# augustgw/early-exit-transformer

Hardware: AMD Instinct MI355X
Metric: mel-frames/sec encoder forward (all exits) + summed per-exit CTC loss, d_model=256 12-layer (higher is better)
Workload: dtype fp16x3 (hi/lo-split fp16 MFMA operands, three products per GEMM, fp32 accumulate; v_mfma_f32_16x16x32_f16)

## Files before the change

### early_exit_transformer_amd/csrc/eec_device.h

```cpp
#pragma once
#include <hip/hip_runtime.h>
#include <stdint.h>

namespace eec {

typedef _Float16 half_t;
typedef _Float16 h8 __attribute__((ext_vector_type(8)));
typedef _Float16 h4 __attribute__((ext_vector_type(4)));
typedef _Float16 h2 __attribute__((ext_vector_type(2)));
typedef float f32x16 __attribute__((ext_vector_type(16)));
typedef float f32x4 __attribute__((ext_vector_type(4)));

#ifndef EEC_OPERAND_BF16
#define EEC_OPERAND_BF16 0
#endif
typedef __bf16 bf8_t __attribute__((ext_vector_type(8)));
typedef __bf16 bf2_t __attribute__((ext_vector_type(2)));
typedef float f32x2_t __attribute__((ext_vector_type(2)));

constexpr int kWave = 64;
constexpr float kLnEps = 1e-5f;
constexpr float kLog2e = 1.4426950408889634f;
constexpr float kHalfMax = 65504.0f;

// ... 318 lines not shown
template <int MT, int NT>
__device__ __forceinline__ void accs_q_to_std(f32x16 (&acc)[MT][NT]) {
  asm volatile("s_nop 7\n\ts_nop 7\n\ts_nop 2" ::: "memory");
#pragma unroll
  for (int a = 0; a < MT; ++a)
#pragma unroll
    for (int b = 0; b < NT; ++b) acc_q_to_std(acc[a][b]);
}
template <int MT, int NT>
__device__ __forceinline__ void accs_std_to_q(f32x16 (&acc)[MT][NT]) {
#pragma unroll
  for (int a = 0; a < MT; ++a)
#pragma unroll
    for (int b = 0; b < NT; ++b) acc_std_to_q(acc[a][b]);
}
__device__ __forceinline__ const char* a_lane16(const char* a_lane, int ld_bytes) {
  const int lane = lane_id(), hh = lane >> 5, u = (lane >> 4) & 1;
  return a_lane + u * (16 - 16 * ld_bytes) + hh * 16;
}
__device__ __forceinline__ const uint4* w_lane16(const uint4* w_lane) {
  const int lane = lane_id(), hh = lane >> 5, u = (lane >> 4) & 1;
  return w_lane + 96 * hh + 16 * u;
}

struct WAddr16 {
  const char* base;
  __device__ __forceinline__ uint4 load(size_t uniform_u4) const { return *(const uint4*)(base + uniform_u4 * 16); }
};
__device__ __forceinline__ WAddr16 w_addr16(const uint4* w_lane) {
  const int lane = lane_id(), hh = lane >> 5, u = (lane >> 4) & 1;
  return WAddr16{(const char*)(w_lane + 96 * hh + 16 * u)};
}

template <int NP, int PF, int NT>
__device__ __forceinline__ void ring_fill_16(WRing<NP, PF, NT>& r, const uint4* __restrict__ w_lane, size_t nt_stride, int steps_avail) {
  static_assert(PF % 2 == 0, "the ring is dealt in double k-steps");
  const WAddr16 w16 = w_addr16(w_lane);
#pragma unroll
  for (int p = 0; p < PF; ++p)
    if (p < steps_avail) {
#pragma unroll
      for (int nt = 0; nt < NT; ++nt) {
        r.q[p][nt][0] = w16.load(nt * nt_stride + 16 * (p & 1) + (size_t)(p >> 1) * 256);
        if (NP == 3) r.q[p][nt][(NP == 3) ? 1 : 0] = w16.load(nt * nt_stride + 16 * (p & 1) + (size_t)(p >> 1) * 256 + 64);
      }
    }
  __builtin_amdgcn_sched_barrier(0);
}

__device__ __forceinline__ void quad_mac16(f32x16& acc, int ra, int cb, h8 a, h8 b) {
  const int q = 4 * (2 * ra + cb);
  f32x4 t = {acc[q], acc[q + 1], acc[q + 2], acc[q + 3]};
  t = mfma32(a, b, t);
  acc[q] = t[0], acc[q + 1] = t[1], acc[q + 2] = t[2], acc[q + 3] = t[3];
}
template <int NP, int KS, int NT, bool SWAP, int PF, typename Side = NoSide, int SIDE_VALU = 0, int MT = 2, bool IN_STD = true, bool OUT_STD = true>
__device__ __forceinline__ void gemm_ring_16(f32x16 (&acc)[MT][NT], const char* a_lane, int ld_bytes, int plane_bytes,
                                             const uint4* __restrict__ w_lane, size_t nt_stride, WRing<NP, PF, NT>& r, Side side = Side()) {
  static_assert(KS % 2 == 0 && PF % 2 == 0, "double k-steps");
  constexpr int LO = (NP == 3) ? 1 : 0;
  const char* a16 = a_lane16(a_lane, ld_bytes);
  const WAddr16 w16 = w_addr16(w_lane);
  if constexpr (IN_STD) accs_std_to_q<MT, NT>(acc);
  h8 ah[2][MT], al[2][MT];
#pragma unroll
  for (int mt = 0; mt < MT; ++mt) {
    ah[0][mt] = *(const h8*)(a16 + mt * 32 * ld_bytes);
    if (NP == 3) al[0][mt] = *(const h8*)(a16 + plane_bytes + mt * 32 * ld_bytes);
  }
#pragma unroll
  for (int p = 0; p < KS; ++p) {
    const int S = p >> 1, rb = p & 1, cur = p & 1, nxt = cur ^ 1;
    if (p + 1 < KS) {
      const int off = (16 * ((p + 1) & 1)) * ld_bytes + ((p + 1) >> 1) * 64;
#pragma unroll
      for (int mt = 0; mt < MT; ++mt) {
        ah[nxt][mt] = *(const h8*)(a16 + mt * 32 * ld_bytes + off);
        if (NP == 3) al[nxt][mt] = *(const h8*)(a16 + plane_bytes + mt * 32 * ld_bytes + off);
      }
      __builtin_amdgcn_sched_barrier(0);
    }
#pragma unroll
    for (int wb = 0; wb < 2; ++wb) {
#pragma unroll
      for (int nt = 0; nt < NT; ++nt) {
        const h8 bh = __builtin_bit_cast(h8, r.q[(2 * S + wb) % PF][nt][0]);
        const h8 bl = __builtin_bit_cast(h8, r.q[(2 * S + wb) % PF][nt][LO]);
#pragma unroll
        for (int pr = (NP == 3 ? 0 : 2); pr < 3; ++pr)
#pragma unroll
          for (int mt = 0; mt < MT; ++mt) {
            const h8 a = pr == 0 ? al[cur][mt] : ah[cur][mt], w = pr == 1 ? bl : bh;
            if (!SWAP) quad_mac16(acc[mt][nt], rb, wb, a, w);
            else quad_mac16(acc[mt][nt], wb, rb, w, a);
          }
        if (rb == 1) {
          if (2 * S + PF < KS) {
            r.q[(2 * S + wb) % PF][nt][0] = w16.load(nt * nt_stride + 16 * wb + (size_t)(S + PF / 2) * 256);
            if (NP == 3) r.q[(2 * S + wb) % PF][nt][LO] = w16.load(nt * nt_stride + 16 * wb + (size_t)(S + PF / 2) * 256 + 64);
          }
        }
      }
    }
    side(p);
    if (SIDE_VALU > 0) {
#pragma unroll
      for (int i = 0; i < MT * NT * NP; ++i) {
        __builtin_amdgcn_sched_group_barrier(0x008, 2, 0);
        __builtin_amdgcn_sched_group_barrier(0x002, SIDE_VALU, 0);
      }
    }
    __builtin_amdgcn_sched_barrier(0);
#ifdef EEC_KSTEP_STAMPS
    if (NT == 2) eec_kstep_stamp();
#endif
  }
  if constexpr (OUT_STD) accs_q_to_std<MT, NT>(acc);
}

template <int NP, int NT, bool SWAP, int MT = 2, bool IN_STD = true, bool OUT_STD = true>
__device__ __forceinline__ void gemm_plain_16(f32x16 (&acc)[MT][NT], const char* a_lane, int ld_bytes, int plane_bytes,
                                              const uint4* __restrict__ w_lane, size_t nt_stride, int ks) {
  const char* a16 = a_lane16(a_lane, ld_bytes);
  const uint4* w16 = w_lane16(w_lane);
  if constexpr (IN_STD) accs_std_to_q<MT, NT>(acc);
  for (int S = 0; S < ks / 2; ++S) {
#pragma unroll
    for (int nt = 0; nt < NT; ++nt) {
      h8 bh[2], bl[2];
#pragma unroll
      for (int rb = 0; rb < 2; ++rb) {
        bh[rb] = __builtin_bit_cast(h8, w16[nt * nt_stride + 16 * rb + (size_t)S * 256]);
        bl[rb] = bh[rb];
        if (NP == 3) bl[rb] = __builtin_bit_cast(h8, w16[nt * nt_stride + 16 * rb + (size_t)S * 256 + 64]);
      }
#pragma unroll
      for (int mt = 0; mt < MT; ++mt) {
        h8 ah[2], al[2];
#pragma unroll
        for (int rb = 0; rb < 2; ++rb) {
          ah[rb] = *(const h8*)(a16 + (mt * 32 + 16 * rb) * ld_bytes + S * 64);
          al[rb] = ah[rb];
          if (NP == 3) al[rb] = *(const h8*)(a16 + plane_bytes + (mt * 32 + 16 * rb) * ld_bytes + S * 64);
        }
        if (NP == 3) {
          if (SWAP) tile_mac16(acc[mt][nt], bh, al), tile_mac16(acc[mt][nt], bl, ah);
          else tile_mac16(acc[mt][nt], al, bh), tile_mac16(acc[mt][nt], ah, bl);
        }
        if (SWAP) tile_mac16(acc[mt][nt], bh, ah);
        else tile_mac16(acc[mt][nt], ah, bh);
      }
    }
  }
  if constexpr (OUT_STD) accs_q_to_std<MT, NT>(acc);
}

template <int NP>
constexpr bool kMfma16For = NP == 3 || (EEC_MFMA16_NP1 != 0 && NP == 1);
template <int NP, int PF, int NT>
__device__ __forceinline__ void ring_fill(WRing<NP, PF, NT>& r, const uint4* __restrict__ w_lane, size_t nt_stride, int steps_avail) {
  if constexpr (kMfma16For<NP>) ring_fill_16<NP, PF, NT>(r, w_lane, nt_stride, steps_avail);
  else ring_fill_32<NP, PF, NT>(r, w_lane, nt_stride, steps_avail);
}
template <int NP, int KS, int NT, bool SWAP, int PF, typename Side = NoSide, int SIDE_VALU = 0, int MT = 2, bool IN_STD = true, bool OUT_STD = true>
__device__ __forceinline__ void gemm_ring(f32x16 (&acc)[MT][NT], const char* a_lane, int ld_bytes, int plane_bytes,
                                          const uint4* __restrict__ w_lane, size_t nt_stride, WRing<NP, PF, NT>& r, Side side = Side()) {
  if constexpr (kMfma16For<NP>) gemm_ring_16<NP, KS, NT, SWAP, PF, Side, SIDE_VALU, MT, IN_STD, OUT_STD>(acc, a_lane, ld_bytes, plane_bytes, w_lane, nt_stride, r, side);
  else gemm_ring_32<NP, KS, NT, SWAP, PF, Side, SIDE_VALU, MT>(acc, a_lane, ld_bytes, plane_bytes, w_lane, nt_stride, r, side);
}
template <int NP, int NT, bool SWAP, int MT = 2, bool IN_STD = true, bool OUT_STD = true>
__device__ __forceinline__ void gemm_plain(f32x16 (&acc)[MT][NT], const char* a_lane, int ld_bytes, int plane_bytes,
                                           const uint4* __restrict__ w_lane, size_t nt_stride, int ks) {
  if constexpr (kMfma16For<NP>) gemm_plain_16<NP, NT, SWAP, MT, IN_STD, OUT_STD>(acc, a_lane, ld_bytes, plane_bytes, w_lane, nt_stride, ks);
  else gemm_plain_32<NP, NT, SWAP, MT>(acc, a_lane, ld_bytes, plane_bytes, w_lane, nt_stride, ks);
}

typedef int i32x8 __attribute__((ext_vector_type(8)));
constexpr int kE8M0One = 127;
constexpr float kF8WLoGain = 1.09f;
constexpr float kF8ALoGain = 1.17f;
__device__ __forceinline__ h2 lo8_gain(h2 lo) {
  const h2 g = {(half_t)kF8ALoGain, (half_t)kF8ALoGain};
  return lo * g;
}

__device__ __forceinline__ uint2 top_bytes(uint4 f) {
  return make_uint2(__builtin_amdgcn_perm(f.y, f.x, 0x07050301u), __builtin_amdgcn_perm(f.w, f.z, 0x07050301u));
}
__device__ __forceinline__ f32x16 mfma_f8(i32x8 a, i32x8 b, f32x16 c, int scale_a, int scale_b) {
  return __builtin_amdgcn_mfma_scale_f32_32x32x64_f8f6f4(a, b, c, 1 , 1 , 0, scale_a, 0, scale_b);
}
__device__ __forceinline__ int lo8_pos(int k) {
  return (k & ~63) + 32 * ((k >> 3) & 1) + 8 * ((k >> 4) & 3) + (k & 7);
}

constexpr int kF8Rec = 400;
template <int NT>
struct WGroupF8 {
  uint4 lo[NT][2];
  int sc[NT];
// ... 304 lines not shown
```

### early_exit_transformer_amd/csrc/ffn.hip

```cpp
#ifdef EEC_FFN_TRAIN_BWD
#define EEC_OPERAND_BF16 1
#endif
#if defined(EEC_FFN_TRAIN) || defined(EEC_FFN_TRAIN_BWD)
#define EEC_MFMA16_NP1 1
#endif
#include "eec_blocks.h"
#include "eec_drop.h"

namespace eec {

constexpr int kFfnThreads = 512;
constexpr int kFC = 128;
constexpr int kHLd = (kFC + 8) * 2;
template <int D>
struct FfnGeo {
  using G = Geo<D>;
  static constexpr int kHPlane = G::kRows * kHLd;
  static constexpr int kNT2 = D / 128;
  static constexpr int kLds = 2 * G::kAPlane + (4 * kHPlane > G::kETile ? 4 * kHPlane : G::kETile);
};
#ifndef EEC_TR_NT
#define EEC_TR_NT 1
#endif
#if defined(EEC_FFN_TRAIN_BWD) && !defined(EEC_PF1_NP3)
// ... 148 lines not shown
  const int lane = lane_id(), w = wave_id();
  const int hh = lane >> 5, wl = w & 3;
  const int w_s = wave_id_sgpr();
  const int wl_s = w_s & 3;
  const bool is_producer = w < 4;
  const int row0 = row_tile_index() * G::kRows;
  const int M = a.M, F = a.F;
  float* __restrict__ x = a.x;
  char* lds_h = smem + 2 * kAPlane;
  char* lds_e = lds_h;
  const char* a_lane = smem + (lane & 31) * kALd + hh * 16;

  const int nft = F / 32;
  const int nchunk = (nft + 3) / 4;
  const int ks2_total = F / 16;
#ifndef EEC_SKEW
#define EEC_SKEW 56
#endif
#ifndef EEC_WARM_SLOTS
#define EEC_WARM_SLOTS 4
#endif
  auto phys = [&](int c) { return c >= nchunk ? c - nchunk : c; };
  const size_t w2_nt_stride = (size_t)ks2_total * 128;

#ifdef EEC_TIMELINE
  int tl_idx = 0;
#endif
  TL_STAMP();
#if EEC_SKEW > 0
  for (int i = 0; i < (int)((blockIdx.x >> 3) & 3); ++i) __builtin_amdgcn_s_sleep(EEC_SKEW);
#endif
  constexpr int RNP = NP == 8 ? 1 : NP;
  constexpr bool Q16 = kMfma16For<NP>;
  auto run = [&](auto prod_tag) {
  constexpr bool producer = decltype(prod_tag)::value;
  [[maybe_unused]] const eect::DropState ds_act(eect::Drop{TR ? a.tr.p : 0.0f, a.tr.seed, a.tr.site_act});
  WRing<RNP, kPF1, 1> r1;
  WRing<RNP, kPF2, NTP> r2;
  WGroupF8<1> wg1[kNW1];
  WGroupF8<NTP> wg2[kNW2];
  const size_t w2f8_nt = (size_t)(F / 64) * kF8Rec;
  auto w1f8_lane = [&](const WPtrs& W, int ft) { return W.w1f8 + (size_t)ft * (D / 64) * kF8Rec + lane; };
  auto w2f8_lane = [&](const WPtrs& W, int c, int h = 0) {
    return W.w2f8 + ((size_t)(NT2 * wl + NTP * h) * (F / 64) + 2 * c) * kF8Rec + lane;
  };
  auto fill1 = [&](const WPtrs& W, int ft) {
    if constexpr (NP == 8) {
      ring_fill_f8<kPF1, 1>(r1, w1f8_lane(W, ft), 0);
#pragma unroll
      for (int g = 0; g < kNW1; ++g) f8_group_load<1>(wg1[g], w1f8_lane(W, ft) + (size_t)g * kF8Rec, 0);
    } else {
      ring_fill<RNP, kPF1, 1>(r1, W.w1p + (size_t)ft * nts + lane, 0, KS);
    }
  };
  auto fill2 = [&](const WPtrs& W, int c) {
    if constexpr (NP == 8) {
      ring_fill_f8<kPF2, NTP>(r2, w2f8_lane(W, c), w2f8_nt);
#pragma unroll
      for (int g = 0; g < kNW2; ++g) f8_group_load<NTP>(wg2[g], w2f8_lane(W, c) + (size_t)g * kF8Rec, w2f8_nt);
    } else {
      ring_fill<RNP, kPF2, NTP>(r2, W.w2p + ((size_t)(NT2 * wl) * ks2_total + c * (kFC / 16)) * 128 + lane, w2_nt_stride,
                             min(kFC / 16, ks2_total - c * (kFC / 16)));
    }
  };
  auto start_streams = [&](const WPtrs& W) {
    if constexpr (producer) {
// ... 128 lines not shown
        const int row = row0 + w * RPW + i;
        v[i] = zero_row<G::kQ>();
        if (row < M) v[i] = load_row<D>(x + (size_t)row * D, lane);
      }
      __builtin_amdgcn_sched_barrier(0);
      start_streams(W0);
      float mu[RPW], rs[RPW];
      layer_norm_rows<D, RPW>(v, lg, lb, mu, rs);
#pragma unroll
      for (int i = 0; i < RPW; ++i) {
        const int row = row0 + w * RPW + i;
        if (row < M) {
          store_row<D>(a.tr.ln + (size_t)row * D, v[i], lane);
          if (lane == 0) a.tr.mean[row] = mu[i], a.tr.rstd[row] = rs[i];
        }
      }
      rows_to_planes<D, NP, RPW>(smem, v, w * RPW, row0, M, true);
    } else {
      rows_f32_to_planes<D, NP, true>(smem, x, row0, M, a.st[0].ln_g, a.st[0].ln_b, [&]() { start_streams(W0); });
    }
  }
  TL_STAMP();
  __syncthreads();
  TL_STAMP();

  [[maybe_unused]] ProjStream<(QNP ? QNP : 1), kLPF, NW> rq;
  unsigned sink = 0;
  const int nslots = nchunk + 2;
  f32x16 acc2c[NH][MT][NTP];
  static_for<NS>([&](auto si_tag) {
    constexpr int si = decltype(si_tag)::value;
    const WPtrs W = wptrs(si);
    const float* __restrict__ b1s = EEC_STAGE_FIELD(si, b1);
    if constexpr (producer) {
      [[maybe_unused]] f32x16 preq[TR == 2 ? MT : 1];
      [[maybe_unused]] auto request_pre = [&](int hcol0) {
#pragma unroll
        for (int mt = 0; mt < MT; ++mt)
#pragma unroll
          for (int g = 0; g < 4; ++g) {
            const int frame = Q16 ? mt * 32 + 16 * (g & 1) + (lane & 15) : mt * 32 + (lane & 31);
            const int hid = Q16 ? wl * 32 + 16 * (g >> 1) + 8 * hh + 4 * ((lane >> 4) & 1) : wl * 32 + 4 * hh + g * 8;
            const int row = min(row0 + frame, M - 1);
            typedef float f32x4_t __attribute__((ext_vector_type(4)));
            const f32x4_t v = __builtin_nontemporal_load((const f32x4_t*)(a.tr.pre + (size_t)row * F + hcol0 + hid));
            preq[mt][4 * g] = v[0], preq[mt][4 * g + 1] = v[1], preq[mt][4 * g + 2] = v[2], preq[mt][4 * g + 3] = v[3];
          }
      };
      auto silu_pair = [&](const f32x16 (&acc)[MT][1], char* hb, int step, h2& keep_hi, h2& keep_lo, [[maybe_unused]] int hcol0 = 0) {
        const int mt = step >> 3, q = step & 7;
        const float u0 = acc[mt][0][2 * q], u1 = acc[mt][0][2 * q + 1];
        if constexpr (TR == 2) {
          const float x0 = preq[mt][2 * q], x1 = preq[mt][2 * q + 1];
          const float sg0 = __builtin_amdgcn_rcpf(1.0f + __builtin_amdgcn_exp2f(-kLog2e * x0));
          const float sg1 = __builtin_amdgcn_rcpf(1.0f + __builtin_amdgcn_exp2f(-kLog2e * x1));
          const float t0 = u0 * sg0 * (1.0f + x0 * (1.0f - sg0)), t1 = u1 * sg1 * (1.0f + x1 * (1.0f - sg1));
          if ((q & 1) == 0) {
            keep_hi = __builtin_bit_cast(h2, t0);
            keep_lo = __builtin_bit_cast(h2, t1);
            return;
          }
          const int g = q >> 1;
          const int frame = Q16 ? mt * 32 + 16 * (g & 1) + (lane & 15) : mt * 32 + (lane & 31);
          const int hid = Q16 ? wl * 32 + 16 * (g >> 1) + 8 * hh + 4 * ((lane >> 4) & 1) : wl * 32 + 4 * hh + g * 8;
          const int row = row0 + frame;
          const size_t idx = (size_t)row * F + hcol0 + hid;
          float m[4];
          ds_act.mul4(idx, m);
          const float d0 = __builtin_bit_cast(float, keep_hi) * m[0], d1 = __builtin_bit_cast(float, keep_lo) * m[1], d2 = t0 * m[2], d3 = t1 * m[3];
          if (row < M) tape_store4(a.tr.act + idx, d0, d1, d2, d3);
          constexpr int SNPT = NP == 1 ? 1 : 3;
          const hl2_t sa = split2<SNPT>(d0, d1), sb = split2<SNPT>(d2, d3);
          char* dst = hb + frame * kHLd + hid * 2;
          h4 hi, lo;
          hi.xy = sa.hi, hi.zw = sb.hi, lo.xy = sa.lo, lo.zw = sb.lo;
          *(h4*)dst = hi;
          if (NP == 3) *(h4*)(dst + kHPlane) = lo;
          return;
        }
        if constexpr (TR == 1) {
          const float s0 = silu_f(u0), s1 = silu_f(u1);
          if ((q & 1) == 0) {
            keep_hi = __builtin_bit_cast(h2, s0);
            keep_lo = __builtin_bit_cast(h2, s1);
            return;
          }
          const int g = q >> 1;
          const int frame = Q16 ? mt * 32 + 16 * (g & 1) + (lane & 15) : mt * 32 + (lane & 31);
          const int hid = Q16 ? wl * 32 + 16 * (g >> 1) + 8 * hh + 4 * ((lane >> 4) & 1) : wl * 32 + 4 * hh + g * 8;
          const int row = row0 + frame;
          const size_t idx = (size_t)row * F + hcol0 + hid;
          float m[4];
          ds_act.mul4(idx, m);
          const float h0 = __builtin_bit_cast(float, keep_hi) * m[0], h1 = __builtin_bit_cast(float, keep_lo) * m[1], h2v = s0 * m[2], h3 = s1 * m[3];
          if (row < M) {
            tape_store4(a.tr.pre + idx, acc[mt][0][2 * q - 2], acc[mt][0][2 * q - 1], u0, u1);
            tape_store4(a.tr.act + idx, h0, h1, h2v, h3);
          }
          constexpr int SNPT = NP == 1 ? 1 : 3;
          const hl2_t sa = split2<SNPT>(h0, h1), sb = split2<SNPT>(h2v, h3);
          char* dst = hb + frame * kHLd + hid * 2;
          h4 hi, lo;
          hi.xy = sa.hi, hi.zw = sb.hi, lo.xy = sa.lo, lo.zw = sb.lo;
          *(h4*)dst = hi;
          if (NP == 3) *(h4*)(dst + kHPlane) = lo;
          return;
        }
        constexpr int SNP = NP == 1 ? 1 : 3;
        const hl2_t sp = ACT == 0 ? split2<SNP>(silu_exp2(u0), silu_exp2(u1)) : split2<SNP>(fmaxf(u0, 0.f), fmaxf(u1, 0.f));
        if ((q & 1) == 0) {
          keep_hi = sp.hi;
          keep_lo = sp.lo;
        } else {
          const int g = q >> 1;
          const int frame = Q16 ? mt * 32 + 16 * (g & 1) + (lane & 15) : mt * 32 + (lane & 31);
          const int hid = Q16 ? wl * 32 + 16 * (g >> 1) + 8 * hh + 4 * ((lane >> 4) & 1) : wl * 32 + 4 * hh + g * 8;
          char* dst = hb + frame * kHLd + hid * 2;
          h4 hi, lo;
          hi.xy = keep_hi, hi.zw = sp.hi, lo.xy = keep_lo, lo.zw = sp.lo;
          *(h4*)dst = hi;
          if (NP == 3) *(h4*)(dst + kHPlane) = lo;
          if (NP == 8) {
            h4 lg;
            lg.xy = lo8_gain(keep_lo), lg.zw = lo8_gain(sp.lo);
            const uint2 lb = __builtin_bit_cast(uint2, lg);
            *(unsigned*)(hb + kHPlane + (mt * 32 + (lane & 31)) * kH8Ld + lo8_pos(wl * 32 + 4 * hh + (q >> 1) * 8)) =
                __builtin_amdgcn_perm(lb.y, lb.x, 0x07050301u);
          }
        }
      };
      auto init_bias = [&](f32x16 (&acc)[MT][1], int ft) {
        if constexpr (TR == 2) {
          zero_acc(acc);
          return;
        }
        if constexpr (Q16) {
          const int u = (lane >> 4) & 1;
#pragma unroll
          for (int ra = 0; ra < 2; ++ra) {
            const float4 bb = *(const float4*)(b1s + ft * 32 + 16 * ra + 8 * hh + 4 * u);
#pragma unroll
            for (int mt = 0; mt < MT; ++mt)
#pragma unroll
              for (int cb = 0; cb < 2; ++cb) {
                acc[mt][0][4 * (2 * ra + cb) + 0] = bb.x;
                acc[mt][0][4 * (2 * ra + cb) + 1] = bb.y;
                acc[mt][0][4 * (2 * ra + cb) + 2] = bb.z;
                acc[mt][0][4 * (2 * ra + cb) + 3] = bb.w;
              }
          }
          return;
        }
#pragma unroll
        for (int g = 0; g < 4; ++g) {
          const float4 bb = *(const float4*)(b1s + ft * 32 + 8 * g + 4 * hh);
#pragma unroll
          for (int mt = 0; mt < MT; ++mt) {
            acc[mt][0][4 * g + 0] = bb.x;
            acc[mt][0][4 * g + 1] = bb.y;
            acc[mt][0][4 * g + 2] = bb.z;
            acc[mt][0][4 * g + 3] = bb.w;
          }
        }
      };
      constexpr int kSideEvery = KS / (8 * MT);
      auto slot = [&](int s, f32x16 (&cur)[MT][1], f32x16 (&prev)[MT][1]) {
        const int ft = (s < nchunk ? phys(s) : s) * 4 + wl;
        const bool do_gemm = s < nchunk && ft < nft;
        const bool do_silu = s >= 1 && s - 1 < nchunk && phys(s - 1) * 4 + wl < nft;
        char* hb_prev = lds_h + ((s - 1) & 1) * 2 * kHPlane;
        [[maybe_unused]] const int hcol_prev = do_silu ? phys(s - 1) * kFC : 0;
        h2 khi, klo;
        if (do_gemm) {
          init_bias(cur, ft);
          const uint4* w1_lane = W.w1p + (size_t)ft * nts + lane;
          const char* a8_lane = smem + kAPlane + (lane & 31) * kA8Ld + hh * 32;
          if (do_silu) {
            auto side = [&](int st) {
              if (st % kSideEvery == 0) silu_pair(prev, hb_prev, st / kSideEvery, khi, klo, hcol_prev);
            };
            if constexpr (NP == 8)
              gemm_ring_f8<D / 64, 1, true, kPF1, decltype(side), EEC_SIDE_VALU_NP8, kNW1, MT>(
                  cur, a_lane, kALd, a8_lane, kA8Ld, w1f8_lane(W, ft), 0, r1, wg1, side);
            else
              gemm_ring<RNP, KS, 1, true, kPF1, decltype(side), (NP == 3 ? EEC_SIDE_VALU_NP3 : 7), MT, !Q16, !Q16>(cur, a_lane, kALd, kAPlane, w1_lane,
                                                                                                  0, r1, side);
          } else {
            if constexpr (NP == 8)
              gemm_ring_f8<D / 64, 1, true, kPF1, NoSide, 0, kNW1, MT>(cur, a_lane, kALd, a8_lane, kA8Ld,
                                                                                                                    w1f8_lane(W, ft), 0, r1, wg1);
            else
              gemm_ring<RNP, KS, 1, true, kPF1, NoSide, 0, MT, !Q16, !Q16>(cur, a_lane, kALd, kAPlane, w1_lane, 0, r1);
          }
          if (s + 1 < nchunk && phys(s + 1) * 4 + wl < nft) fill1(W, phys(s + 1) * 4 + wl);
          if constexpr (TR == 2) request_pre(phys(s) * kFC);
        } else if (do_silu) {
#pragma unroll
          for (int st = 0; st < 8 * MT; ++st) silu_pair(prev, hb_prev, st, khi, klo, hcol_prev);
        }
        TL_STAMP();
        __syncthreads();
        TL_STAMP();
      };
      f32x16 accA[MT][1], accB[MT][1];
      for (int s = 0; s < nslots; s += 2) {
        slot(s, accA, accB);
        if (s + 1 < nslots) slot(s + 1, accB, accA);
      }
    } else {
#pragma unroll
      for (int h = 0; h < NH; ++h) zero_acc(acc2c[h]);
#if EEC_WARM_SLOTS > 0
      unsigned warm[4] = {0u, 0u, 0u, 0u};
#endif
      for (int s = 0; s < nslots; ++s) {
#if EEC_WARM_SLOTS > 0
        if (s == nslots - EEC_WARM_SLOTS) {
          const int lane_t = fresh_lane();
          if constexpr (si + 1 < NS) {
            const WPtrs Wn = wptrs(si + 1);
            const size_t wbytes = NP == 8 ? (size_t)(F / 32) * (D / 64) * kF8Rec * 16 : (size_t)F * D * 2 * (NP == 3 ? 2 : 1);
#pragma unroll
            for (int j = 0; j < 2; ++j) {
              warm[j] = touch_share(NP == 8 ? (const void*)Wn.w1f8 : (const void*)Wn.w1p, wbytes, wl_s, j, lane_t);
              warm[2 + j] = touch_share(NP == 8 ? (const void*)Wn.w2f8 : (const void*)Wn.w2p, wbytes, wl_s, j, lane_t);
            }
          } else if constexpr (QNP != 0) {
            warm[0] = QNP == 8 ? touch_share(a.qkv.wf8, (size_t)(3 * D / 32) * (D / 64) * kF8Rec * 16, wl_s, 0, lane_t)
                               : touch_share(a.qkv.wp, (size_t)3 * D * D * 2 * (QNP == 3 ? 2 : 1), wl_s, 0, lane_t);
          }
        }
#endif
        if (s >= 2) {
          const int cl = s - 2, c = phys(cl);
          const char* h_lane = lds_h + (cl & 1) * 2 * kHPlane + (lane & 31) * kHLd + hh * 16;
          const int ks2 = min(kFC / 16, ks2_total - c * (kFC / 16));
          const uint4* w2_lane = W.w2p + ((size_t)(NT2 * wl) * ks2_total + c * (kFC / 16)) * 128 + lane;
          if constexpr (NP == 8) {
            const char* h8_lane = lds_h + (cl & 1) * 2 * kHPlane + kHPlane + (lane & 31) * kH8Ld + hh * 32;
            if constexpr (NH == 1) {
              gemm_ring_f8<2, NTP, false, kPF2, NoSide, 0, kNW2, MT>(acc2c[0], h_lane, kHLd, h8_lane, kH8Ld, w2f8_lane(W, c), w2f8_nt, r2, wg2);
            } else {
#pragma unroll
              for (int h = 0; h < NH; ++h) {
                const uint4* next = h + 1 < NH ? w2f8_lane(W, c, h + 1) : (cl + 1 < nchunk ? w2f8_lane(W, phys(cl + 1), 0) : nullptr);
                gemm_ring_f8<2, NTP, false, kPF2, NoSide, 0, kNW2, MT, true>(acc2c[h], h_lane, kHLd, h8_lane, kH8Ld, w2f8_lane(W, c, h), w2f8_nt, r2, wg2, NoSide(), next);
              }
            }
          } else if (ks2 == kFC / 16) {
            gemm_ring<RNP, kFC / 16, NTP, false, kPF2, NoSide, 0, MT, !Q16, !Q16>(acc2c[0], h_lane, kHLd, kHPlane, w2_lane, w2_nt_stride, r2);
          } else {
            gemm_plain<RNP, NTP, false, MT, !Q16, !Q16>(acc2c[0], h_lane, kHLd, kHPlane, w2_lane, w2_nt_stride, ks2);
          }
          if (NH == 1 && cl + 1 < nchunk) fill2(W, phys(cl + 1));
        }
        TL_STAMP();
        __syncthreads();
        TL_STAMP();
      }
#if EEC_WARM_SLOTS > 0
      sink ^= warm[0] ^ warm[1] ^ warm[2] ^ warm[3];
#endif
    }
    const int lane_e = fresh_lane(), w_e = w_s;
    RowV<G::kQ> xr[RPW];
#pragma unroll
    for (int i = 0; i < RPW; ++i) {
      const int row = row0 + w_e * RPW + i;
      xr[i] = zero_row<G::kQ>();
      if (TR != 2 && row < M) xr[i] = load_row<D>(x + (size_t)row * D, lane_e);
    }
    __builtin_amdgcn_sched_barrier(0);
    constexpr bool more = si + 1 < NS;
    TL_STAMP();
    if constexpr (!producer) {
      if constexpr (Q16) {
#pragma unroll
        for (int h = 0; h < NH; ++h) accs_q_to_std<MT, NTP>(acc2c[h]);
      }
#pragma unroll
      for (int h = 0; h < NH; ++h)
        acc_to_etile<MT, NTP>(lds_e, G::kELd, acc2c[h], wl_s * 32 * NT2 + h * 32 * NTP, EEC_STAGE_FIELD(si, b2), lane_e);
    }
    TL_STAMP();
    if constexpr (more) {
      start_streams(wptrs(1));
    } else if constexpr (QNP != 0) {
      proj_fill<D, QNP, kLPF, NW>(rq, WMat{a.qkv.wp, a.qkv.wf8}, NW * w);
    }
    __syncthreads();
    TL_STAMP();
// ... 240 lines not shown
```

Baseline: 19.03 million.

## Split first FFN chunk's GEMM1 across producer and consumer waves by weight half

Adds a WBM mask to the 16x16x32 ring GEMM so a caller can compute only one half of the weight row-blocks. In the FFN kernel's fp16x3 path, the first slot's up-projection is split: producer waves compute the even half while consumer waves, which would otherwise sit idle during the first two slots, compute the odd half and apply SiLU to their part of the hidden tile. This is meant to shorten the pipeline fill latency at the start of each stage. The cost is more code paths, extra registers in the consumer, and an extra split of the SiLU work and sync logic, which could raise register pressure.

```diff
diff --git a/early_exit_transformer_amd/csrc/eec_device.h b/early_exit_transformer_amd/csrc/eec_device.h
--- a/early_exit_transformer_amd/csrc/eec_device.h
+++ b/early_exit_transformer_amd/csrc/eec_device.h
@@ -374,13 +374,13 @@
   return WAddr16{(const char*)(w_lane + 96 * hh + 16 * u)};
 }
 
-template <int NP, int PF, int NT>
+template <int NP, int PF, int NT, int WBM = 3>
 __device__ __forceinline__ void ring_fill_16(WRing<NP, PF, NT>& r, const uint4* __restrict__ w_lane, size_t nt_stride, int steps_avail) {
   static_assert(PF % 2 == 0, "the ring is dealt in double k-steps");
   const WAddr16 w16 = w_addr16(w_lane);
 #pragma unroll
   for (int p = 0; p < PF; ++p)
-    if (p < steps_avail) {
+    if (((WBM >> (p & 1)) & 1) && p < steps_avail) {
 #pragma unroll
       for (int nt = 0; nt < NT; ++nt) {
         r.q[p][nt][0] = w16.load(nt * nt_stride + 16 * (p & 1) + (size_t)(p >> 1) * 256);
@@ -396,7 +396,8 @@
   t = mfma32(a, b, t);
   acc[q] = t[0], acc[q + 1] = t[1], acc[q + 2] = t[2], acc[q + 3] = t[3];
 }
-template <int NP, int KS, int NT, bool SWAP, int PF, typename Side = NoSide, int SIDE_VALU = 0, int MT = 2, bool IN_STD = true, bool OUT_STD = true>
+template <int NP, int KS, int NT, bool SWAP, int PF, typename Side = NoSide, int SIDE_VALU = 0, int MT = 2, bool IN_STD = true, bool OUT_STD = true,
+          int WBM = 3>
 __device__ __forceinline__ void gemm_ring_16(f32x16 (&acc)[MT][NT], const char* a_lane, int ld_bytes, int plane_bytes,
                                              const uint4* __restrict__ w_lane, size_t nt_stride, WRing<NP, PF, NT>& r, Side side = Side()) {
   static_assert(KS % 2 == 0 && PF % 2 == 0, "double k-steps");
@@ -424,6 +425,7 @@
     }
 #pragma unroll
     for (int wb = 0; wb < 2; ++wb) {
+      if (!((WBM >> wb) & 1)) continue;
 #pragma unroll
       for (int nt = 0; nt < NT; ++nt) {
         const h8 bh = __builtin_bit_cast(h8, r.q[(2 * S + wb) % PF][nt][0]);
@@ -447,7 +449,7 @@
     side(p);
     if (SIDE_VALU > 0) {
 #pragma unroll
-      for (int i = 0; i < MT * NT * NP; ++i) {
+      for (int i = 0; i < MT * NT * NP * (WBM == 3 ? 2 : 1) / 2; ++i) {
         __builtin_amdgcn_sched_group_barrier(0x008, 2, 0);
         __builtin_amdgcn_sched_group_barrier(0x002, SIDE_VALU, 0);
       }
@@ -499,15 +501,18 @@
 
 template <int NP>
 constexpr bool kMfma16For = NP == 3 || (EEC_MFMA16_NP1 != 0 && NP == 1);
-template <int NP, int PF, int NT>
+template <int NP, int PF, int NT, int WBM = 3>
 __device__ __forceinline__ void ring_fill(WRing<NP, PF, NT>& r, const uint4* __restrict__ w_lane, size_t nt_stride, int steps_avail) {
-  if constexpr (kMfma16For<NP>) ring_fill_16<NP, PF, NT>(r, w_lane, nt_stride, steps_avail);
+  static_assert(WBM == 3 || kMfma16For<NP>, "weight row-block halves: 16x16x32 forms only");
+  if constexpr (kMfma16For<NP>) ring_fill_16<NP, PF, NT, WBM>(r, w_lane, nt_stride, steps_avail);
   else ring_fill_32<NP, PF, NT>(r, w_lane, nt_stride, steps_avail);
 }
-template <int NP, int KS, int NT, bool SWAP, int PF, typename Side = NoSide, int SIDE_VALU = 0, int MT = 2, bool IN_STD = true, bool OUT_STD = true>
+template <int NP, int KS, int NT, bool SWAP, int PF, typename Side = NoSide, int SIDE_VALU = 0, int MT = 2, bool IN_STD = true, bool OUT_STD = true,
+          int WBM = 3>
 __device__ __forceinline__ void gemm_ring(f32x16 (&acc)[MT][NT], const char* a_lane, int ld_bytes, int plane_bytes,
                                           const uint4* __restrict__ w_lane, size_t nt_stride, WRing<NP, PF, NT>& r, Side side = Side()) {
-  if constexpr (kMfma16For<NP>) gemm_ring_16<NP, KS, NT, SWAP, PF, Side, SIDE_VALU, MT, IN_STD, OUT_STD>(acc, a_lane, ld_bytes, plane_bytes, w_lane, nt_stride, r, side);
+  static_assert(WBM == 3 || kMfma16For<NP>, "weight row-block halves: 16x16x32 forms only");
+  if constexpr (kMfma16For<NP>) gemm_ring_16<NP, KS, NT, SWAP, PF, Side, SIDE_VALU, MT, IN_STD, OUT_STD, WBM>(acc, a_lane, ld_bytes, plane_bytes, w_lane, nt_stride, r, side);
   else gemm_ring_32<NP, KS, NT, SWAP, PF, Side, SIDE_VALU, MT>(acc, a_lane, ld_bytes, plane_bytes, w_lane, nt_stride, r, side);
 }
 template <int NP, int NT, bool SWAP, int MT = 2, bool IN_STD = true, bool OUT_STD = true>
diff --git a/early_exit_transformer_amd/csrc/ffn.hip b/early_exit_transformer_amd/csrc/ffn.hip
--- a/early_exit_transformer_amd/csrc/ffn.hip
+++ b/early_exit_transformer_amd/csrc/ffn.hip
@@ -204,6 +204,8 @@
 #endif
   constexpr int RNP = NP == 8 ? 1 : NP;
   constexpr bool Q16 = kMfma16For<NP>;
+  constexpr bool kShare = NP == 3 && TR == 0 && MT == 2;
+  const bool share = kShare && F % kFC == 0 && nchunk >= 4;
   auto run = [&](auto prod_tag) {
   constexpr bool producer = decltype(prod_tag)::value;
   [[maybe_unused]] const eect::DropState ds_act(eect::Drop{TR ? a.tr.p : 0.0f, a.tr.seed, a.tr.site_act});
@@ -398,142 +400,150 @@
     constexpr int si = decltype(si_tag)::value;
     const WPtrs W = wptrs(si);
     const float* __restrict__ b1s = EEC_STAGE_FIELD(si, b1);
-    if constexpr (producer) {
-      [[maybe_unused]] f32x16 preq[TR == 2 ? MT : 1];
-      [[maybe_unused]] auto request_pre = [&](int hcol0) {
-#pragma unroll
-        for (int mt = 0; mt < MT; ++mt)
-#pragma unroll
-          for (int g = 0; g < 4; ++g) {
-            const int frame = Q16 ? mt * 32 + 16 * (g & 1) + (lane & 15) : mt * 32 + (lane & 31);
-            const int hid = Q16 ? wl * 32 + 16 * (g >> 1) + 8 * hh + 4 * ((lane >> 4) & 1) : wl * 32 + 4 * hh + g * 8;
-            const int row = min(row0 + frame, M - 1);
-            typedef float f32x4_t __attribute__((ext_vector_type(4)));
-            const f32x4_t v = __builtin_nontemporal_load((const f32x4_t*)(a.tr.pre + (size_t)row * F + hcol0 + hid));
-            preq[mt][4 * g] = v[0], preq[mt][4 * g + 1] = v[1], preq[mt][4 * g + 2] = v[2], preq[mt][4 * g + 3] = v[3];
-          }
-      };
-      auto silu_pair = [&](const f32x16 (&acc)[MT][1], char* hb, int step, h2& keep_hi, h2& keep_lo, [[maybe_unused]] int hcol0 = 0) {
-        const int mt = step >> 3, q = step & 7;
-        const float u0 = acc[mt][0][2 * q], u1 = acc[mt][0][2 * q + 1];
-        if constexpr (TR == 2) {
-          const float x0 = preq[mt][2 * q], x1 = preq[mt][2 * q + 1];
-          const float sg0 = __builtin_amdgcn_rcpf(1.0f + __builtin_amdgcn_exp2f(-kLog2e * x0));
-          const float sg1 = __builtin_amdgcn_rcpf(1.0f + __builtin_amdgcn_exp2f(-kLog2e * x1));
-          const float t0 = u0 * sg0 * (1.0f + x0 * (1.0f - sg0)), t1 = u1 * sg1 * (1.0f + x1 * (1.0f - sg1));
-          if ((q & 1) == 0) {
-            keep_hi = __builtin_bit_cast(h2, t0);
-            keep_lo = __builtin_bit_cast(h2, t1);
-            return;
-          }
-          const int g = q >> 1;
+    [[maybe_unused]] f32x16 preq[TR == 2 ? MT : 1];
+    [[maybe_unused]] auto request_pre = [&](int hcol0) {
+#pragma unroll
+      for (int mt = 0; mt < MT; ++mt)
+#pragma unroll
+        for (int g = 0; g < 4; ++g) {
           const int frame = Q16 ? mt * 32 + 16 * (g & 1) + (lane & 15) : mt * 32 + (lane & 31);
           const int hid = Q16 ? wl * 32 + 16 * (g >> 1) + 8 * hh + 4 * ((lane >> 4) & 1) : wl * 32 + 4 * hh + g * 8;
-          const int row = row0 + frame;
-          const size_t idx = (size_t)row * F + hcol0 + hid;
-          float m[4];
-          ds_act.mul4(idx, m);
-          const float d0 = __builtin_bit_cast(float, keep_hi) * m[0], d1 = __builtin_bit_cast(float, keep_lo) * m[1], d2 = t0 * m[2], d3 = t1 * m[3];
-          if (row < M) tape_store4(a.tr.act + idx, d0, d1, d2, d3);
-          constexpr int SNPT = NP == 1 ? 1 : 3;
-          const hl2_t sa = split2<SNPT>(d0, d1), sb = split2<SNPT>(d2, d3);
-          char* dst = hb + frame * kHLd + hid * 2;
-          h4 hi, lo;
-          hi.xy = sa.hi, hi.zw = sb.hi, lo.xy = sa.lo, lo.zw = sb.lo;
-          *(h4*)dst = hi;
-          if (NP == 3) *(h4*)(dst + kHPlane) = lo;
+          const int row = min(row0 + frame, M - 1);
+          typedef float f32x4_t __attribute__((ext_vector_type(4)));
+          const f32x4_t v = __builtin_nontemporal_load((const f32x4_t*)(a.tr.pre + (size_t)row * F + hcol0 + hid));
+          preq[mt][4 * g] = v[0], preq[mt][4 * g + 1] = v[1], preq[mt][4 * g + 2] = v[2], preq[mt][4 * g + 3] = v[3];
+        }
+    };
+    auto silu_pair = [&](const f32x16 (&acc)[MT][1], char* hb, int step, h2& keep_hi, h2& keep_lo, [[maybe_unused]] int hcol0 = 0) {
+      const int mt = step >> 3, q = step & 7;
+      const float u0 = acc[mt][0][2 * q], u1 = acc[mt][0][2 * q + 1];
+      if constexpr (TR == 2) {
+        const float x0 = preq[mt][2 * q], x1 = preq[mt][2 * q + 1];
+        const float sg0 = __builtin_amdgcn_rcpf(1.0f + __builtin_amdgcn_exp2f(-kLog2e * x0));
+        const float sg1 = __builtin_amdgcn_rcpf(1.0f + __builtin_amdgcn_exp2f(-kLog2e * x1));
+        const float t0 = u0 * sg0 * (1.0f + x0 * (1.0f - sg0)), t1 = u1 * sg1 * (1.0f + x1 * (1.0f - sg1));
+        if ((q & 1) == 0) {
+          keep_hi = __builtin_bit_cast(h2, t0);
+          keep_lo = __builtin_bit_cast(h2, t1);
           return;
         }
-        if constexpr (TR == 1) {
-          const float s0 = silu_f(u0), s1 = silu_f(u1);
-          if ((q & 1) == 0) {
-            keep_hi = __builtin_bit_cast(h2, s0);
-            keep_lo = __builtin_bit_cast(h2, s1);
-            return;
-          }
-          const int g = q >> 1;
-          const int frame = Q16 ? mt * 32 + 16 * (g & 1) + (lane & 15) : mt * 32 + (lane & 31);
-          const int hid = Q16 ? wl * 32 + 16 * (g >> 1) + 8 * hh + 4 * ((lane >> 4) & 1) : wl * 32 + 4 * hh + g * 8;
-          const int row = row0 + frame;
-          const size_t idx = (size_t)row * F + hcol0 + hid;
-          float m[4];
-          ds_act.mul4(idx, m);
-          const float h0 = __builtin_bit_cast(float, keep_hi) * m[0], h1 = __builtin_bit_cast(float, keep_lo) * m[1], h2v = s0 * m[2], h3 = s1 * m[3];
-          if (row < M) {
-            tape_store4(a.tr.pre + idx, acc[mt][0][2 * q - 2], acc[mt][0][2 * q - 1], u0, u1);
-            tape_store4(a.tr.act + idx, h0, h1, h2v, h3);
-          }
-          constexpr int SNPT = NP == 1 ? 1 : 3;
-          const hl2_t sa = split2<SNPT>(h0, h1), sb = split2<SNPT>(h2v, h3);
-          char* dst = hb + frame * kHLd + hid * 2;
-          h4 hi, lo;
-          hi.xy = sa.hi, hi.zw = sb.hi, lo.xy = sa.lo, lo.zw = sb.lo;
-          *(h4*)dst = hi;
-          if (NP == 3) *(h4*)(dst + kHPlane) = lo;
+        const int g = q >> 1;
+        const int frame = Q16 ? mt * 32 + 16 * (g & 1) + (lane & 15) : mt * 32 + (lane & 31);
+        const int hid = Q16 ? wl * 32 + 16 * (g >> 1) + 8 * hh + 4 * ((lane >> 4) & 1) : wl * 32 + 4 * hh + g * 8;
+        const int row = row0 + frame;
+        const size_t idx = (size_t)row * F + hcol0 + hid;
+        float m[4];
+        ds_act.mul4(idx, m);
+        const float d0 = __builtin_bit_cast(float, keep_hi) * m[0], d1 = __builtin_bit_cast(float, keep_lo) * m[1], d2 = t0 * m[2], d3 = t1 * m[3];
+        if (row < M) tape_store4(a.tr.act + idx, d0, d1, d2, d3);
+        constexpr int SNPT = NP == 1 ? 1 : 3;
+        const hl2_t sa = split2<SNPT>(d0, d1), sb = split2<SNPT>(d2, d3);
+        char* dst = hb + frame * kHLd + hid * 2;
+        h4 hi, lo;
+        hi.xy = sa.hi, hi.zw = sb.hi, lo.xy = sa.lo, lo.zw = sb.lo;
+        *(h4*)dst = hi;
+        if (NP == 3) *(h4*)(dst + kHPlane) = lo;
+        return;
+      }
+      if constexpr (TR == 1) {
+        const float s0 = silu_f(u0), s1 = silu_f(u1);
+        if ((q & 1) == 0) {
+          keep_hi = __builtin_bit_cast(h2, s0);
+          keep_lo = __builtin_bit_cast(h2, s1);
           return;
         }
-        constexpr int SNP = NP == 1 ? 1 : 3;
-        const hl2_t sp = ACT == 0 ? split2<SNP>(silu_exp2(u0), silu_exp2(u1)) : split2<SNP>(fmaxf(u0, 0.f), fmaxf(u1, 0.f));
-        if ((q & 1) == 0) {
-          keep_hi = sp.hi;
-          keep_lo = sp.lo;
-        } else {
-          const int g = q >> 1;
-          const int frame = Q16 ? mt * 32 + 16 * (g & 1) + (lane & 15) : mt * 32 + (lane & 31);
-          const int hid = Q16 ? wl * 32 + 16 * (g >> 1) + 8 * hh + 4 * ((lane >> 4) & 1) : wl * 32 + 4 * hh + g * 8;
-          char* dst = hb + frame * kHLd + hid * 2;
-          h4 hi, lo;
-          hi.xy = keep_hi, hi.zw = sp.hi, lo.xy = keep_lo, lo.zw = sp.lo;
-          *(h4*)dst = hi;
-          if (NP == 3) *(h4*)(dst + kHPlane) = lo;
-          if (NP == 8) {
-            h4 lg;
-            lg.xy = lo8_gain(keep_lo), lg.zw = lo8_gain(sp.lo);
-            const uint2 lb = __builtin_bit_cast(uint2, lg);
-            *(unsigned*)(hb + kHPlane + (mt * 32 + (lane & 31)) * kH8Ld + lo8_pos(wl * 32 + 4 * hh + (q >> 1) * 8)) =
-                __builtin_amdgcn_perm(lb.y, lb.x, 0x07050301u);
-          }
-        }
+        const int g = q >> 1;
+        const int frame = Q16 ? mt * 32 + 16 * (g & 1) + (lane & 15) : mt * 32 + (lane & 31);
+        const int hid = Q16 ? wl * 32 + 16 * (g >> 1) + 8 * hh + 4 * ((lane >> 4) & 1) : wl * 32 + 4 * hh + g * 8;
+        const int row = row0 + frame;
+        const size_t idx = (size_t)row * F + hcol0 + hid;
+        float m[4];
+        ds_act.mul4(idx, m);
+        const float h0 = __builtin_bit_cast(float, keep_hi) * m[0], h1 = __builtin_bit_cast(float, keep_lo) * m[1], h2v = s0 * m[2], h3 = s1 * m[3];
+        if (row < M) {
+          tape_store4(a.tr.pre + idx, acc[mt][0][2 * q - 2], acc[mt][0][2 * q - 1], u0, u1);
+          tape_store4(a.tr.act + idx, h0, h1, h2v, h3);
+        }
+        constexpr int SNPT = NP == 1 ? 1 : 3;
+        const hl2_t sa = split2<SNPT>(h0, h1), sb = split2<SNPT>(h2v, h3);
+        char* dst = hb + frame * kHLd + hid * 2;
+        h4 hi, lo;
+        hi.xy = sa.hi, hi.zw = sb.hi, lo.xy = sa.lo, lo.zw = sb.lo;
+        *(h4*)dst = hi;
+        if (NP == 3) *(h4*)(dst + kHPlane) = lo;
+        return;
+      }
+      constexpr int SNP = NP == 1 ? 1 : 3;
+      const hl2_t sp = ACT == 0 ? split2<SNP>(silu_exp2(u0), silu_exp2(u1)) : split2<SNP>(fmaxf(u0, 0.f), fmaxf(u1, 0.f));
+      if ((q & 1) == 0) {
+        keep_hi = sp.hi;
+        keep_lo = sp.lo;
+      } else {
+        const int g = q >> 1;
+        const int frame = Q16 ? mt * 32 + 16 * (g & 1) + (lane & 15) : mt * 32 + (lane & 31);
+        const int hid = Q16 ? wl * 32 + 16 * (g >> 1) + 8 * hh + 4 * ((lane >> 4) & 1) : wl * 32 + 4 * hh + g * 8;
+        char* dst = hb + frame * kHLd + hid * 2;
+        h4 hi, lo;
+        hi.xy = keep_hi, hi.zw = sp.hi, lo.xy = keep_lo, lo.zw = sp.lo;
+        *(h4*)dst = hi;
+        if (NP == 3) *(h4*)(dst + kHPlane) = lo;
+        if (NP == 8) {
+          h4 lg;
+          lg.xy = lo8_gain(keep_lo), lg.zw = lo8_gain(sp.lo);
+          const uint2 lb = __builtin_bit_cast(uint2, lg);
+          *(unsigned*)(hb + kHPlane + (mt * 32 + (lane & 31)) * kH8Ld + lo8_pos(wl * 32 + 4 * hh + (q >> 1) * 8)) =
+              __builtin_amdgcn_perm(lb.y, lb.x, 0x07050301u);
+        }
+      }
+    };
+    auto init_bias = [&](f32x16 (&acc)[MT][1], int ft) {
+      if constexpr (TR == 2) {
+        zero_acc(acc);
+        return;
+      }
+      if constexpr (Q16) {
+        const int u = (lane >> 4) & 1;
+#pragma unroll
+        for (int ra = 0; ra < 2; ++ra) {
+          const float4 bb = *(const float4*)(b1s + ft * 32 + 16 * ra + 8 * hh + 4 * u);
+#pragma unroll
+          for (int mt = 0; mt < MT; ++mt)
+#pragma unroll
+            for (int cb = 0; cb < 2; ++cb) {
+              acc[mt][0][4 * (2 * ra + cb) + 0] = bb.x;
+              acc[mt][0][4 * (2 * ra + cb) + 1] = bb.y;
+              acc[mt][0][4 * (2 * ra + cb) + 2] = bb.z;
+              acc[mt][0][4 * (2 * ra + cb) + 3] = bb.w;
+            }
+        }
+        return;
+      }
+#pragma unroll
+      for (int g = 0; g < 4; ++g) {
+        const float4 bb = *(const float4*)(b1s + ft * 32 + 8 * g + 4 * hh);
+#pragma unroll
+        for (int mt = 0; mt < MT; ++mt) {
+          acc[mt][0][4 * g + 0] = bb.x;
+          acc[mt][0][4 * g + 1] = bb.y;
+          acc[mt][0][4 * g + 2] = bb.z;
+          acc[mt][0][4 * g + 3] = bb.w;
+        }
+      }
+    };
+    constexpr int kSideEvery = KS / (8 * MT);
+    auto half_step = [](int j, int wb) { return (j >> 2) * 8 + 4 * wb + (j & 3); };
+    if constexpr (producer) {
+      auto slot_end = [&]() {
+        TL_STAMP();
+        __syncthreads();
+        TL_STAMP();
       };
-      auto init_bias = [&](f32x16 (&acc)[MT][1], int ft) {
-        if constexpr (TR == 2) {
-          zero_acc(acc);
-          return;
-        }
-        if constexpr (Q16) {
-          const int u = (lane >> 4) & 1;
-#pragma unroll
-          for (int ra = 0; ra < 2; ++ra) {
-            const float4 bb = *(const float4*)(b1s + ft * 32 + 16 * ra + 8 * hh + 4 * u);
-#pragma unroll
-            for (int mt = 0; mt < MT; ++mt)
-#pragma unroll
-              for (int cb = 0; cb < 2; ++cb) {
-                acc[mt][0][4 * (2 * ra + cb) + 0] = bb.x;
-                acc[mt][0][4 * (2 * ra + cb) + 1] = bb.y;
-                acc[mt][0][4 * (2 * ra + cb) + 2] = bb.z;
-                acc[mt][0][4 * (2 * ra + cb) + 3] = bb.w;
-              }
-          }
-          return;
-        }
-#pragma unroll
-        for (int g = 0; g < 4; ++g) {
-          const float4 bb = *(const float4*)(b1s + ft * 32 + 8 * g + 4 * hh);
-#pragma unroll
-          for (int mt = 0; mt < MT; ++mt) {
-            acc[mt][0][4 * g + 0] = bb.x;
-            acc[mt][0][4 * g + 1] = bb.y;
-            acc[mt][0][4 * g + 2] = bb.z;
-            acc[mt][0][4 * g + 3] = bb.w;
-          }
-        }
-      };
-      constexpr int kSideEvery = KS / (8 * MT);
-      auto slot = [&](int s, f32x16 (&cur)[MT][1], f32x16 (&prev)[MT][1]) {
+      auto slot = [&](int s, f32x16 (&cur)[MT][1], f32x16 (&prev)[MT][1], auto fill_tag) {
+        constexpr bool FILL = decltype(fill_tag)::value;
         const int ft = (s < nchunk ? phys(s) : s) * 4 + wl;
         const bool do_gemm = s < nchunk && ft < nft;
         const bool do_silu = s >= 1 && s - 1 < nchunk && phys(s - 1) * 4 + wl < nft;
+        const bool half_g = FILL && s == 0, half_s = FILL && s == 1;
         char* hb_prev = lds_h + ((s - 1) & 1) * 2 * kHPlane;
         [[maybe_unused]] const int hcol_prev = do_silu ? phys(s - 1) * kFC : 0;
         h2 khi, klo;
@@ -545,9 +555,18 @@
             auto side = [&](int st) {
               if (st % kSideEvery == 0) silu_pair(prev, hb_prev, st / kSideEvery, khi, klo, hcol_prev);
             };
+            auto side_h = [&](int st) {
+              if (st % (2 * kSideEvery) == 0) silu_pair(prev, hb_prev, half_step(st / (2 * kSideEvery), 0), khi, klo);
+            };
             if constexpr (NP == 8)
               gemm_ring_f8<D / 64, 1, true, kPF1, decltype(side), EEC_SIDE_VALU_NP8, kNW1, MT>(
                   cur, a_lane, kALd, a8_lane, kA8Ld, w1f8_lane(W, ft), 0, r1, wg1, side);
+            else if (kShare && half_g)
+              gemm_ring<RNP, KS, 1, true, kPF1, decltype(side_h), EEC_SIDE_VALU_NP3, MT, !Q16, !Q16, kShare ? 1 : 3>(
+                  cur, a_lane, kALd, kAPlane, w1_lane, 0, r1, side_h);
+            else if (kShare && half_s)
+              gemm_ring<RNP, KS, 1, true, kPF1, decltype(side_h), EEC_SIDE_VALU_NP3, MT, !Q16, !Q16>(cur, a_lane, kALd, kAPlane, w1_lane, 0, r1,
+                                                                                                   side_h);
             else
               gemm_ring<RNP, KS, 1, true, kPF1, decltype(side), (NP == 3 ? EEC_SIDE_VALU_NP3 : 7), MT, !Q16, !Q16>(cur, a_lane, kALd, kAPlane, w1_lane,
                                                                                                   0, r1, side);
@@ -555,31 +574,45 @@
             if constexpr (NP == 8)
               gemm_ring_f8<D / 64, 1, true, kPF1, NoSide, 0, kNW1, MT>(cur, a_lane, kALd, a8_lane, kA8Ld,
                                                                                                                     w1f8_lane(W, ft), 0, r1, wg1);
+            else if (kShare && half_g)
+              gemm_ring<RNP, KS, 1, true, kPF1, NoSide, 0, MT, !Q16, !Q16, kShare ? 1 : 3>(cur, a_lane, kALd, kAPlane, w1_lane, 0, r1);
             else
               gemm_ring<RNP, KS, 1, true, kPF1, NoSide, 0, MT, !Q16, !Q16>(cur, a_lane, kALd, kAPlane, w1_lane, 0, r1);
           }
           if (s + 1 < nchunk && phys(s + 1) * 4 + wl < nft) fill1(W, phys(s + 1) * 4 + wl);
           if constexpr (TR == 2) request_pre(phys(s) * kFC);
         } else if (do_silu) {
-#pragma unroll
-          for (int st = 0; st < 8 * MT; ++st) silu_pair(prev, hb_prev, st, khi, klo, hcol_prev);
-        }
+          if (kShare && half_s) {
+#pragma unroll
+            for (int j = 0; j < 4 * MT; ++j) silu_pair(prev, hb_prev, half_step(j, 0), khi, klo);
+          } else {
+#pragma unroll
+            for (int st = 0; st < 8 * MT; ++st) silu_pair(prev, hb_prev, st, khi, klo, hcol_prev);
+          }
+        }
+        slot_end();
+      };
+      f32x16 accA[MT][1], accB[MT][1];
+      int s_begin = 0;
+      if (kShare && share) {
+        slot(0, accA, accB, BoolTag<kShare>{});
+        slot(1, accB, accA, BoolTag<kShare>{});
+        s_begin = 2;
+      }
+      for (int s = s_begin; s < nslots; s += 2) {
+        slot(s, accA, accB, BoolTag<false>{});
+        if (s + 1 < nslots) slot(s + 1, accB, accA, BoolTag<false>{});
+      }
+    } else {
+      auto slot_end = [&]() {
         TL_STAMP();
         __syncthreads();
         TL_STAMP();
       };
-      f32x16 accA[MT][1], accB[MT][1];
-      for (int s = 0; s < nslots; s += 2) {
-        slot(s, accA, accB);
-        if (s + 1 < nslots) slot(s + 1, accB, accA);
-      }
-    } else {
-#pragma unroll
-      for (int h = 0; h < NH; ++h) zero_acc(acc2c[h]);
 #if EEC_WARM_SLOTS > 0
       unsigned warm[4] = {0u, 0u, 0u, 0u};
 #endif
-      for (int s = 0; s < nslots; ++s) {
+      auto warm_up = [&](int s) {
 #if EEC_WARM_SLOTS > 0
         if (s == nslots - EEC_WARM_SLOTS) {
           const int lane_t = fresh_lane();
@@ -597,32 +630,52 @@
           }
         }
 #endif
-        if (s >= 2) {
-          const int cl = s - 2, c = phys(cl);
-          const char* h_lane = lds_h + (cl & 1) * 2 * kHPlane + (lane & 31) * kHLd + hh * 16;
-          const int ks2 = min(kFC / 16, ks2_total - c * (kFC / 16));
-          const uint4* w2_lane = W.w2p + ((size_t)(NT2 * wl) * ks2_total + c * (kFC / 16)) * 128 + lane;
-          if constexpr (NP == 8) {
-            const char* h8_lane = lds_h + (cl & 1) * 2 * kHPlane + kHPlane + (lane & 31) * kH8Ld + hh * 32;
-            if constexpr (NH == 1) {
-              gemm_ring_f8<2, NTP, false, kPF2, NoSide, 0, kNW2, MT>(acc2c[0], h_lane, kHLd, h8_lane, kH8Ld, w2f8_lane(W, c), w2f8_nt, r2, wg2);
-            } else {
-#pragma unroll
-              for (int h = 0; h < NH; ++h) {
-                const uint4* next = h + 1 < NH ? w2f8_lane(W, c, h + 1) : (cl + 1 < nchunk ? w2f8_lane(W, phys(cl + 1), 0) : nullptr);
-                gemm_ring_f8<2, NTP, false, kPF2, NoSide, 0, kNW2, MT, true>(acc2c[h], h_lane, kHLd, h8_lane, kH8Ld, w2f8_lane(W, c, h), w2f8_nt, r2, wg2, NoSide(), next);
-              }
+      };
+      auto gemm2 = [&](int s) {
+        const int cl = s - 2, c = phys(cl);
+        const char* h_lane = lds_h + (cl & 1) * 2 * kHPlane + (lane & 31) * kHLd + hh * 16;
+        const int ks2 = min(kFC / 16, ks2_total - c * (kFC / 16));
+        const uint4* w2_lane = W.w2p + ((size_t)(NT2 * wl) * ks2_total + c * (kFC / 16)) * 128 + lane;
+        if constexpr (NP == 8) {
+          const char* h8_lane = lds_h + (cl & 1) * 2 * kHPlane + kHPlane + (lane & 31) * kH8Ld + hh * 32;
+          if constexpr (NH == 1) {
+            gemm_ring_f8<2, NTP, false, kPF2, NoSide, 0, kNW2, MT>(acc2c[0], h_lane, kHLd, h8_lane, kH8Ld, w2f8_lane(W, c), w2f8_nt, r2, wg2);
+          } else {
+#pragma unroll
+            for (int h = 0; h < NH; ++h) {
+              const uint4* next = h + 1 < NH ? w2f8_lane(W, c, h + 1) : (cl + 1 < nchunk ? w2f8_lane(W, phys(cl + 1), 0) : nullptr);
+              gemm_ring_f8<2, NTP, false, kPF2, NoSide, 0, kNW2, MT, true>(acc2c[h], h_lane, kHLd, h8_lane, kH8Ld, w2f8_lane(W, c, h), w2f8_nt, r2, wg2, NoSide(), next);
             }
-          } else if (ks2 == kFC / 16) {
-            gemm_ring<RNP, kFC / 16, NTP, false, kPF2, NoSide, 0, MT, !Q16, !Q16>(acc2c[0], h_lane, kHLd, kHPlane, w2_lane, w2_nt_stride, r2);
-          } else {
-            gemm_plain<RNP, NTP, false, MT, !Q16, !Q16>(acc2c[0], h_lane, kHLd, kHPlane, w2_lane, w2_nt_stride, ks2);
           }
-          if (NH == 1 && cl + 1 < nchunk) fill2(W, phys(cl + 1));
-        }
-        TL_STAMP();
-        __syncthreads();
-        TL_STAMP();
+        } else if (ks2 == kFC / 16) {
+          gemm_ring<RNP, kFC / 16, NTP, false, kPF2, NoSide, 0, MT, !Q16, !Q16>(acc2c[0], h_lane, kHLd, kHPlane, w2_lane, w2_nt_stride, r2);
+        } else {
+          gemm_plain<RNP, NTP, false, MT, !Q16, !Q16>(acc2c[0], h_lane, kHLd, kHPlane, w2_lane, w2_nt_stride, ks2);
+        }
+        if (NH == 1 && cl + 1 < nchunk) fill2(W, phys(cl + 1));
+      };
+      int s0 = 0;
+      if constexpr (kShare) {
+        if (share) {
+          f32x16 hA[MT][1];
+          h2 khi, klo;
+          WRing<RNP, kPF1, 1> hr;
+          ring_fill<RNP, kPF1, 1, 2>(hr, W.w1p + (size_t)wl * nts + lane, 0, KS);
+          init_bias(hA, wl);
+          gemm_ring<RNP, KS, 1, true, kPF1, NoSide, 0, MT, false, false, 2>(hA, a_lane, kALd, kAPlane, W.w1p + (size_t)wl * nts + lane, 0, hr);
+          slot_end();
+#pragma unroll
+          for (int j = 0; j < 4 * MT; ++j) silu_pair(hA, lds_h, half_step(j, 1), khi, klo);
+          slot_end();
+          s0 = 2;
+        }
+      }
+#pragma unroll
+      for (int h = 0; h < NH; ++h) zero_acc(acc2c[h]);
+      for (int s = s0; s < nslots; ++s) {
+        warm_up(s);
+        if (s >= 2) gemm2(s);
+        slot_end();
       }
 #if EEC_WARM_SLOTS > 0
       sink ^= warm[0] ^ warm[1] ^ warm[2] ^ warm[3];
```

After: 18.95 million, median of 6. No clear change (-0.4%).
